# google-deepmind/bsuite

Measured on AMD Instinct MI355X. Metric: env-steps/sec, higher is better.
Workload: dtype int32; 1 GPU; deep_sea/10 deep_sea {'size': 30, 'mapping_seed': 42} random actions, dense TimeStep; mode=e, lanes_per_gpu=1048576, global_lanes=1048576, episode_phases=staggered

## Files before the change

bsuite_amd/_native.py:

```python
import ctypes
import os

import torch

_HERE = os.path.dirname(os.path.abspath(__file__))
SO_PATH = os.path.join(_HERE, '_lib', 'libbsuite_amd.so')

FIRST, MID, LAST = 0, 1, 2
BSX_EINVAL, BSX_ENULL, BSX_EALIGN, BSX_ERANGE, BSX_EMODE, BSX_ENOMEM = -1, -2, -3, -4, -5, -6
WRAP_NONE, WRAP_SCALE, WRAP_NOISE, WRAP_SCALE_NOISE, WRAP_NOISE_SCALE = 0, 1, 2, 3, 4
COUNTER_SHARDS, COUNTER_STRIDE = 256, 16
DEEP_SEA_MAX_SIZE = 64
BANDIT_MAX_ACTIONS = 32
FUSED_CATCH_MAX_CELLS = 128


class NativeLibraryError(RuntimeError):
  pass


def _load():
  override = os.environ.get('BSX_NATIVE_LIB')
  if override:
    try:
# ... 171 lines not shown


class ImageCfg(ctypes.Structure):
  _fields_ = [('mode', ctypes.c_int32), ('in_rows', ctypes.c_int32), ('in_cols', ctypes.c_int32),
              ('out_rows', ctypes.c_int32), ('out_cols', ctypes.c_int32), ('tail', ctypes.c_int32),
              ('radius_y', ctypes.c_int32), ('radius_x', ctypes.c_int32),
              ('gauss_y', ctypes.c_double * (IMAGE_MAX_RADIUS + 1)),
              ('gauss_x', ctypes.c_double * (IMAGE_MAX_RADIUS + 1))]


lib = _load()

_P = ctypes.c_void_p
_SIGS = {
    'bsx_abi_version': ([], ctypes.c_int),
    'bsx_observation_dtypes': ([ctypes.c_int32], ctypes.c_int),
    'bsx_observation_index_width': ([ctypes.c_int32], ctypes.c_int),
    'bsx_row_scratch_bytes': ([ctypes.c_int32, ctypes.c_int32, ctypes.c_int64], ctypes.c_int64),
    'bsx_bsuite_info': ([ctypes.c_int32, ctypes.c_int32, ctypes.c_int64, _P, _P, ctypes.c_int32, ctypes.c_int32, _P, _P],
                        ctypes.c_int),
    'bsx_lane_reset_mark': ([ctypes.c_int32, ctypes.c_int32, ctypes.c_int64, _P, _P, _P, ctypes.c_int32, _P], ctypes.c_int),
    'bsx_strerror': ([ctypes.c_int], ctypes.c_char_p),
    'bsx_calib_fill': ([_P, ctypes.c_int64, ctypes.c_int32, _P], ctypes.c_int),
    'bsx_calib_copy': ([_P, _P, ctypes.c_int64, ctypes.c_int32, _P], ctypes.c_int),
    'bsx_counter_add': ([_P, ctypes.c_uint64, _P], ctypes.c_int),
    'bsx_lambda_returns': ([ctypes.POINTER(Returns), _P], ctypes.c_int),
    'bsx_image_observation': ([ctypes.POINTER(ImageCfg), ctypes.c_int64, _P, _P, _P], ctypes.c_int),
    'bsx_image_observation_typed': ([ctypes.POINTER(ImageCfg), ctypes.c_int64, _P, ctypes.c_int32, _P, ctypes.c_int32,
                                     _P], ctypes.c_int),
    'bsx_stream_dump': ([ctypes.c_uint64, ctypes.c_uint64, ctypes.c_int64, ctypes.c_uint64,
                         ctypes.c_int32, ctypes.c_int32, _P, _P, _P], ctypes.c_int),
    'bsx_deep_sea_step': ([ctypes.POINTER(DeepSeaCfg), ctypes.POINTER(Call), _P, _P, TimeStepPtrs, _P],
                          ctypes.c_int),
    'bsx_catch_step': ([ctypes.POINTER(CatchCfg), ctypes.POINTER(Call), _P, _P, TimeStepPtrs, _P],
                       ctypes.c_int),
    'bsx_deep_sea_policy_rollout': ([ctypes.POINTER(DeepSeaCfg), ctypes.POINTER(Call), ctypes.POINTER(Policy), _P,
                                     TimeStepPtrs, _P], ctypes.c_int),
    'bsx_catch_policy_rollout': ([ctypes.POINTER(CatchCfg), ctypes.POINTER(Call), ctypes.POINTER(Policy), _P,
                                  TimeStepPtrs, _P], ctypes.c_int),
    'bsx_deep_sea_policy_evaluate': ([ctypes.POINTER(DeepSeaCfg), ctypes.POINTER(Call), ctypes.POINTER(Policy), _P,
                                      PolicyEvalPtrs, _P], ctypes.c_int),
    'bsx_catch_policy_evaluate': ([ctypes.POINTER(CatchCfg), ctypes.POINTER(Call), ctypes.POINTER(Policy), _P,
                                   PolicyEvalPtrs, _P], ctypes.c_int),
    'bsx_deep_sea_policy_sample': ([ctypes.POINTER(DeepSeaCfg), ctypes.POINTER(Call), ctypes.POINTER(PolicyLogits), _P,
                                    TimeStepPtrs, _P], ctypes.c_int),
    'bsx_catch_policy_sample': ([ctypes.POINTER(CatchCfg), ctypes.POINTER(Call), ctypes.POINTER(PolicyLogits), _P,
                                 TimeStepPtrs, _P], ctypes.c_int),
    'bsx_deep_sea_policy_sample_evaluate': ([ctypes.POINTER(DeepSeaCfg), ctypes.POINTER(Call), ctypes.POINTER(PolicyLogits), _P,
                                             PolicyEvalPtrs, _P], ctypes.c_int),
    'bsx_catch_policy_sample_evaluate': ([ctypes.POINTER(CatchCfg), ctypes.POINTER(Call), ctypes.POINTER(PolicyLogits), _P,
                                          PolicyEvalPtrs, _P], ctypes.c_int),
    'bsx_deep_sea_embedding_rollout': ([ctypes.POINTER(DeepSeaCfg), ctypes.POINTER(Call), ctypes.POINTER(PolicyEmbedding), _P,
                                        TimeStepPtrs, _P], ctypes.c_int),
    'bsx_catch_embedding_rollout': ([ctypes.POINTER(CatchCfg), ctypes.POINTER(Call), ctypes.POINTER(PolicyEmbedding), _P,
                                     TimeStepPtrs, _P], ctypes.c_int),
    'bsx_deep_sea_embedding_evaluate': ([ctypes.POINTER(DeepSeaCfg), ctypes.POINTER(Call), ctypes.POINTER(PolicyEmbedding), _P,
                                         PolicyEvalPtrs, _P], ctypes.c_int),
    'bsx_catch_embedding_evaluate': ([ctypes.POINTER(CatchCfg), ctypes.POINTER(Call), ctypes.POINTER(PolicyEmbedding), _P,
                                      PolicyEvalPtrs, _P], ctypes.c_int),
    'bsx_deep_sea_embedding_sample': ([ctypes.POINTER(DeepSeaCfg), ctypes.POINTER(Call), ctypes.POINTER(PolicyEmbeddingSample), _P,
                                       TimeStepPtrs, _P], ctypes.c_int),
    'bsx_catch_embedding_sample': ([ctypes.POINTER(CatchCfg), ctypes.POINTER(Call), ctypes.POINTER(PolicyEmbeddingSample), _P,
                                    TimeStepPtrs, _P], ctypes.c_int),
    'bsx_deep_sea_embedding_sample_evaluate': ([ctypes.POINTER(DeepSeaCfg), ctypes.POINTER(Call), ctypes.POINTER(PolicyEmbeddingSample),
                                                _P, PolicyEvalPtrs, _P], ctypes.c_int),
    'bsx_catch_embedding_sample_evaluate': ([ctypes.POINTER(CatchCfg), ctypes.POINTER(Call), ctypes.POINTER(PolicyEmbeddingSample), _P,
# ... 81 lines not shown
```

bsuite_amd/csrc/deep_sea.hip:

```cpp
#include "bsx_embed_device.h"
#include "bsx_pair_host.h"
#include "bsx_tab_eval.h"
#include "bsx_tab_sample_device.h"
#include "deep_sea_fam.h"
#include "pair_mixed.h"

template <int K>
__global__ void __launch_bounds__(BSX_BLOCK) deep_sea_step1_kernel(const deep_sea_fam::args a, const uint32_t cells,
                                                                   const uint32_t cells_magic, const bsx_div64 dv) {
  __shared__ deep_sea_fam::shared s_map[BSX_BLOCK / BSX_WAVE];
  const int wl = (int)(threadIdx.x & 63u);
  deep_sea_fam::shared& map = s_map[threadIdx.x >> 6];
  const int64_t n_lanes = a.ctl.n_lanes;
  const uint64_t step = bsx_step_of(a.ctl);
  const int32_t tag_new = (int32_t)(((uint32_t)(step + 1) & 1u) << DS_TAG_SHIFT);
  const bool forced = a.ctl.force_reset != 0;
  const deep_sea_hot fn{a.size};
  const uint64_t total = (uint64_t)n_lanes * cells;
  const uint64_t F0 = (uint64_t)blockIdx.x * (uint64_t)(K * 4 * BSX_BLOCK);
  const uint64_t lane_b = __umul64hi(F0, dv.m) >> dv.s;
  const uint32_t r_b = (uint32_t)(F0 - lane_b * cells);
  bsx_f4* __restrict__ o4 = reinterpret_cast<bsx_f4*>(a.out.observation + F0);
  const int32_t* __restrict__ st_b = a.state + lane_b;
  const int32_t* __restrict__ act_b = a.action + (forced ? 0 : lane_b);

  uint32_t dl[K];
  int r0[K];
  bool live[K];
#pragma unroll
  for (int u = 0; u < K; ++u) {
    const uint32_t c = (threadIdx.x >> 6) * (K * 64) + u * 64 + (threadIdx.x & 63);
    const uint32_t f = r_b + (c << 2);
    dl[u] = __umulhi(f, cells_magic);
    r0[u] = (int)(f - dl[u] * cells);
    live[u] = F0 + ((uint64_t)c << 2) + 3 < total;
  }
  const uint32_t dA = dl[0];
  uint32_t dB = dA;
  bool wrA = false, wrB = false;
#pragma unroll
  for (int u = 0; u < K; ++u) {
    if (live[u]) dB = dl[u];
  }
// ... 27 lines not shown
    return nst;
  };
  int tA = -1, tB = -1;
  int32_t nA = 0, nB = 0;
  if (any) {
    nA = resolve(dA, wA, aA, wrA, tA);
    nB = dB != dA ? resolve(dB, wB, aB, wrB, tB) : nA;
  }
  int hA, hB, unused;
  fn(nA, hA, unused);
  fn(nB, hB, unused);
#pragma unroll
  for (int u = 0; u < K; ++u) {
    if (!live[u]) continue;
    int hot = dl[u] == dA ? hA : hB;
    const int p0 = hot < 0 ? -1 : hot - r0[u];
    bsx_f4 v;
    v.x = p0 == 0 ? 1.0f : 0.0f;
    v.y = p0 == 1 ? 1.0f : 0.0f;
    v.z = p0 == 2 ? 1.0f : 0.0f;
    v.w = p0 == 3 ? 1.0f : 0.0f;
    o4[(threadIdx.x >> 6) * (K * 64) + u * 64 + (threadIdx.x & 63)] = v;
  }
  const unsigned int n_last = (unsigned int)__popcll(__ballot(tA == BSX_LAST)) + (unsigned int)__popcll(__ballot(tB == BSX_LAST));
  const unsigned int n_first = (unsigned int)__popcll(__ballot(tA == BSX_FIRST)) + (unsigned int)__popcll(__ballot(tB == BSX_FIRST));
  if (a.ctl.counters != nullptr && wl == 0 && (n_last | n_first) != 0u) {
    unsigned long long* shard = (unsigned long long*)a.ctl.counters +
                                (size_t)((blockIdx.x * (BSX_BLOCK / BSX_WAVE) + (threadIdx.x >> 6)) & (BSX_COUNTER_SHARDS - 1)) * BSX_COUNTER_STRIDE;
    if (n_last) atomicAdd(&shard[0], (unsigned long long)n_last);
    if (n_first) atomicAdd(&shard[1], (unsigned long long)n_first);
  }
}

static int deep_sea_check_cfg(const bsx_deep_sea_t* cfg) {
  return (cfg->size < 1 || cfg->size > BSX_DEEP_SEA_MAX_SIZE) ? BSX_ERANGE : 0;
}

static void deep_sea_fill(const bsx_deep_sea_t* cfg, const bsx_call_t* call, const int32_t* action, int32_t* state,
                          bsx_timestep_t out, double* info, deep_sea_fam::args* a) {
  a->ctl = bsx_make_ctl(call);
  a->action = action; a->state = state; a->out = out; a->info = info;
  a->move_cost = cfg->move_cost; a->inv_size = cfg->inv_size;
  a->size = cfg->size; a->deterministic = cfg->deterministic;
  for (int w = 0; w < DS_MAP_WORDS; ++w) a->mapping_bits[w] = cfg->mapping_bits[w];
}

static int deep_sea_make(const bsx_deep_sea_t* cfg, const bsx_call_t* call, const int32_t* action,
                         int32_t* state, bsx_timestep_t out, double* info, deep_sea_fam::args* a) {
  if (cfg == nullptr) return BSX_ENULL;
  int rc = bsx_check_call(call, action, out, true, true);
  if (rc != 0) return rc;
  if ((rc = deep_sea_check_cfg(cfg)) != 0) return rc;
  if (call->stream.mt_state != nullptr && !cfg->deterministic && call->stream.mt_gauss == nullptr)
    return BSX_ENULL;
  if (call->n_lanes > 0 && (state == nullptr || info == nullptr)) return BSX_ENULL;
  deep_sea_fill(cfg, call, action, state, out, info, a);
  return 0;
}

extern "C" int bsx_deep_sea_step(const bsx_deep_sea_t* cfg, const bsx_call_t* call,
                                 const int32_t* action, int32_t* state, bsx_timestep_t out,
                                 double* info) {
  deep_sea_fam::args a;
  int rc = deep_sea_make(cfg, call, action, state, out, info, &a);
  if (rc != 0) return rc;
  if (call->n_lanes == 0) return 0;
  const uint32_t cells = (uint32_t)(cfg->size * cfg->size);
  static const int step1_env = bsx_env_int("BSX_DEEP_SEA_STEP1", 1);
  if (step1_env != 0 && (int64_t)call->n_lanes * cells * 4 <= ((int64_t)1 << 30) && (call->flags & BSX_CALL_STATE_TAGGED) && call->n_steps <= 1 && call->action_ring <= 1 && cfg->deterministic && bsx_ctl_lean(a.ctl) &&
      call->obs_paint == nullptr && bsx_call_obs(call) == 0 && !bsx_call_index(call) && (cells & 3u) == 0 && cells >= 3u * 256u) {
    constexpr int K = 4;
    const uint64_t total = (uint64_t)call->n_lanes * cells;
    const uint64_t blocks = (total + (uint64_t)K * 4 * BSX_BLOCK - 1) / ((uint64_t)K * 4 * BSX_BLOCK);
    if (blocks > 0x7FFFFFFFull) return BSX_EINVAL;
    deep_sea_step1_kernel<K><<<dim3((unsigned)blocks), dim3(BSX_BLOCK), 0, (hipStream_t)call->hip_stream>>>(
        a, cells, bsx_div_magic(cells), bsx_make_div64(cells));
    return bsx_launch_status();
  }
  return bsx_pair_call<deep_sea_fam, deep_sea_hot, 4>(a, call, action, state, out, cells, deep_sea_hot{cfg->size});
}

extern "C" int bsx_deep_sea_policy_rollout(const bsx_deep_sea_t* cfg, const bsx_call_t* call, const bsx_policy_t* policy,
                                           int32_t* state, bsx_timestep_t out, double* info) {
  if (cfg == nullptr || call == nullptr || policy == nullptr) return BSX_ENULL;
  int rc = deep_sea_check_cfg(cfg);
  if (rc == 0) rc = bsx_check_policy_call(call, policy, bsx_policy_states_deep_sea(cfg->size), state, out, info);
  if (rc != 0 || call->n_lanes == 0) return rc;
  deep_sea_fam::args a;
  rc = deep_sea_make(cfg, call, policy->actions_out, state, out, info, &a);
  if (rc != 0) return rc;
  a.action = nullptr;
  return bsx_policy_rollout_call<deep_sea_fam, deep_sea_hot>(a, call, policy, 2u, out, deep_sea_hot{cfg->size});
}

extern "C" int bsx_deep_sea_policy_evaluate(const bsx_deep_sea_t* cfg, const bsx_call_t* call, const bsx_policy_t* policy,
                                             int32_t* state, bsx_policy_eval_t out, double* info) {
  if (cfg == nullptr || call == nullptr || policy == nullptr) return BSX_ENULL;
  int rc = deep_sea_check_cfg(cfg);
  if (rc == 0) rc = bsx_check_policy_eval_call(call, policy, bsx_policy_states_deep_sea(cfg->size), state, out, info);
  if (rc != 0 || call->n_lanes == 0) return rc;
  bsx_tab_eval_args e;
  deep_sea_fill(cfg, call, nullptr, state, bsx_timestep_t{}, info, &e.fam.deep_sea);
  return bsx_tab_eval_call(e, BSX_FAM_DEEP_SEA, call, policy, 2u, out);
}

extern "C" int bsx_deep_sea_policy_sample(const bsx_deep_sea_t* cfg, const bsx_call_t* call, const bsx_policy_logits_t* policy,
                                          int32_t* state, bsx_timestep_t out, double* info) {
  if (cfg == nullptr || call == nullptr || policy == nullptr) return BSX_ENULL;
  int rc = deep_sea_check_cfg(cfg);
  if (rc == 0) rc = bsx_check_tab_softmax_call(call, policy, bsx_policy_states_deep_sea(cfg->size), 2, state, out, info);
  if (rc != 0 || call->n_lanes == 0) return rc;
  bsx_tab_softmax_args s;
// ... 96 lines not shown
```

bsuite_amd/environments/base.py:

```python
import collections
import contextlib
import ctypes
import math
import secrets
from typing import Any, Dict, Optional

import numpy as np
import torch

from bsuite_amd import _native
from bsuite_amd import dm_env_compat as dm_env
from bsuite_amd.dm_env_compat import specs

_MASK63 = (1 << 63) - 1


_current_raw_stream = getattr(torch._C, '_cuda_getCurrentRawStream', None)
if _current_raw_stream is None:
  def _current_raw_stream(index):
    return torch.cuda.current_stream(index).cuda_stream
_current_device = getattr(torch._C, '_cuda_getDevice', None) or torch.cuda.current_device


_OBS_CODES = {torch.float32: 0, torch.uint8: 1, torch.float16: 2, torch.bfloat16: 3}
# ... 7 lines not shown

_MT_COLUMNS = ('state', 'pos', 'gauss', 'has_gauss')


PolicyEvaluation = collections.namedtuple('PolicyEvaluation', ['episodes', 'return_sum', 'episode_return_sum'])
LinearEvaluation = collections.namedtuple('LinearEvaluation', ['episodes', 'return_sum', 'episode_return_sum', 'observation'])


def raw(env):
  return env.raw_env if hasattr(env, 'raw_env') else env


def _timestep_ptrs(o) -> '_native.TimeStepPtrs':
  return _native.TimeStepPtrs(o['reward'].data_ptr(), o['discount'].data_ptr(), o['step_type'].data_ptr(),
                              o['observation'].data_ptr())


def _resolve_seed(seed: Optional[int]) -> int:
  if seed is None:
    return secrets.randbits(63)
  return int(seed) & _MASK63


class Environment(dm_env.EnvironmentBase):

  bsuite_num_episodes: int

  _supports_delta = False
  _supports_narrow_obs = False
  _index_width = 0
  _pipelined_rollout = False
  scalar_host_buffers = True
  row_path_min_bytes = None
  _state_tag_bit = None
  _state_lib_bits = 0
  _tag_calls = False
  _info_keys = ()
  _info_int_keys = ()
  _abi_name = None
  _cfg = None

  def __init__(self, obs_shape, num_actions, *, seed=None, batch=None, device=None,
               lane_offset=0, num_buffers=2, device_step_counter=False, shared_step_counter=None,
               rng='philox', observation_mode='dense', obs_allocator=None, observation_dtype=torch.float32):
    self._scalar = batch is None
    self._scalar_last_type = None
    self._batch = 1 if batch is None else int(batch)
    if self._batch < 1:
      raise ValueError('batch must be >= 1')
    self._device = torch.device('cuda:0' if device is None else device)
    if self._device.type == 'cuda' and self._device.index is None:
      self._device = torch.device('cuda', torch.cuda.current_device() if torch.cuda.is_available() else 0)
    self._lane_offset = int(lane_offset)
    self._seed = _resolve_seed(seed if seed is None or isinstance(seed, (int, np.integer)) else 0)
    self._obs_shape = tuple(int(d) for d in obs_shape)
    self._num_actions = int(num_actions)
    self._num_buffers = max(1, int(num_buffers))
    self._device_step_counter = bool(device_step_counter) or shared_step_counter is not None
    self._shared_step_counter = shared_step_counter
    self._obs_allocator = obs_allocator
    self._resolve_observations(observation_mode, observation_dtype)
    if rng not in ('philox', 'mt19937'):
      raise ValueError("rng must be 'philox' or 'mt19937'")
    self._rng_mode = rng
    self._mt_seeds = None
    if rng == 'mt19937':
      if seed is None or isinstance(seed, (int, np.integer)):
        self._mt_seeds = [(self._seed + i) & 0xFFFFFFFF for i in range(self._batch)]
      else:
        self._mt_seeds = [int(x) for x in seed]
        if len(self._mt_seeds) != self._batch:
          raise ValueError('need one seed per lane')
    self._wrap = (_native.WRAP_NONE, 0.0, 0, 0.0)
    self._wrap_mt_seeds = None
    self._wrap_mt = None
    self._logging = None
    self._deferred_steps = None
    self._grouped_by = None
    self._rollout_out = {}
    self._policy_rollout_out = {}
    self._policy_eval_out = None
    self._linear_eval_out = None
    self._state_alt = None
    self._row_buf = None
    self._dev_index = self._device.index
    self._step_index = 0
    self._buf = 0
    self._allocated = False
    self._reset_next_step = True

  def _resolve_observations(self, observation_mode, observation_dtype):
    if observation_mode not in ('dense', 'delta', 'index'):
      raise ValueError("observation_mode must be 'dense', 'delta' or 'index'")
    if observation_mode == 'delta' and not self._supports_delta:
      raise ValueError(f'{type(self).__name__} has no delta observation mode (its observations are small and dense)')
    self._delta = observation_mode == 'delta'
    self._index = observation_mode == 'index'
    self._board_shape = self._obs_shape
    if self._index:
      if not self._index_width:
        raise ValueError(f'{type(self).__name__} has no index observation mode (its observations are not one-hot boards)')
      if self._scalar:
        raise ValueError("observation_mode='index' needs the batched view (batch=B)")
      if self._obs_allocator is not None:
        raise ValueError("observation_mode='index' is not available in SweepBatch (float32 arenas)")
    dt = _OBS_NAMES.get(observation_dtype, observation_dtype) if isinstance(observation_dtype, str) else observation_dtype
    if dt not in _OBS_CODES:
      raise ValueError(f'observation_dtype must be one of {sorted(_OBS_NAMES)} (or the torch dtypes), got {observation_dtype!r}')
    if dt != torch.float32:
      if not self._supports_narrow_obs:
        raise ValueError(f'{type(self).__name__} writes float32 observations only (observation_dtype={observation_dtype!r})')
      if self._scalar:
        raise ValueError('observation_dtype other than float32 needs the batched view (batch=B)')
      if self._delta:
        raise ValueError("observation_dtype other than float32 needs observation_mode='dense'")
      if self._obs_allocator is not None:
        raise ValueError('observation_dtype other than float32 is not available in SweepBatch (float32 arenas)')
# ... 59 lines not shown

  def _state_tensors(self) -> Dict[str, torch.Tensor]:
    raise NotImplementedError

  def _native_args(self, call, action_ptr, out):
    state = tuple(t.data_ptr() for t in self._state.values())
    info = (self._info.data_ptr(),) if self._info_keys else ()
    return (ctypes.byref(self._cfg), ctypes.byref(call), action_ptr) + state + (out,) + info

  def _launch(self, call, action_ptr, out) -> int:
    return getattr(_native.lib, f'bsx_{self._abi_name}_step')(*self._native_args(call, action_ptr, out))

  def _group_set(self, group, index: int, action: torch.Tensor, *, out=None, state_alt=None,
                 swap_state: bool = False, row_scratch=None) -> int:
    if self._index:
      raise ValueError("grouped launches write dense observations; use observation_mode='dense'")
    self._ensure_allocated()
    ring = int(action.shape[0]) if (torch.is_tensor(action) and action.dim() == 2) else 0
    if (not torch.is_tensor(action) or action.dtype != torch.int32 or action.device != self._device
        or tuple(action.shape) not in ((self._batch,), (ring, self._batch)) or not action.is_contiguous()
        or (action.dim() == 2 and (ring < 1 or ring & (ring - 1)))):
      raise ValueError(f'grouped launches read the action tensor in place every step: need a contiguous int32 '
                       f'tensor of shape ({self._batch},) — or an action ring (R, {self._batch}) with R a power '
                       f'of two — on {self._device}')
    if not self._device_step_counter:
      raise ValueError('grouped launches need device_step_counter / shared_step_counter')
    if self._delta:
      raise ValueError("grouped launches write dense observations; use observation_mode='dense'")
    if self._obs_flags:
      raise ValueError('grouped launches write float32 observations; use observation_dtype=torch.float32')
    call = self._call_desc
    call.force_reset, call.n_steps = 0, 0
    self._sync_wrap()
    call.stream.step_index = 0
    call.action_ring = ring
    self._buf = 1 % self._num_buffers
    ptrs = self._out_ptrs[0] if out is None else _timestep_ptrs(out)
    own = self._state.get('state')
    own_rows = call.row_scratch
    if row_scratch is not None:
      call.row_scratch = row_scratch.data_ptr() if row_scratch is not False else None
    try:
      if state_alt is not None:
        if swap_state:
          self._state['state'], call.state_alt = state_alt, own.data_ptr()
        else:
          call.state_alt = state_alt.data_ptr()
      return getattr(_native.lib, f'bsx_group_set_{self._abi_name}')(
          group, index, *self._native_args(call, action.data_ptr(), ptrs))
    finally:
      call.state_alt = None
      call.action_ring = 0
      call.row_scratch = own_rows
      if state_alt is not None:
        self._state['state'] = own

  def _row_scratch_words(self) -> int:
    fam = _native.FAMILY_IDS.get(self._abi_name, -1)
    return int(_native.lib.bsx_row_scratch_bytes(fam, int(np.prod(self._obs_shape)), self._batch)) // 4 if fam >= 0 else 0

  def _row_scratch(self, fresh: bool = False) -> Optional[torch.Tensor]:
    words = self._row_scratch_words()
    if not words:
      return None
    if fresh or self._row_buf is None:
      with torch.cuda.device(self._device):
# ... 67 lines not shown
      self._scalar_action = torch.zeros(1, dtype=torch.int32, **place)
      self._reward_f64 = torch.zeros(1, dtype=torch.float64, **place) if self._scalar else None
      self._out_np = [{k: v.numpy() for k, v in o.items()} for o in self._out] if self._host_out else None
    self._mt = None
    if self._rng_mode == 'mt19937':
      with torch.cuda.device(dev):
        self._mt = self._mt_columns(self._mt_seeds, dev, prepare=self._mt_constructor_draws)
    mt_ptrs = [self._mt[k].data_ptr() if self._mt else None for k in _MT_COLUMNS]
    self._call_desc = _native.Call(
        n_lanes=B, force_reset=0,
        stream=_native.Stream(self._seed, self._lane_offset, 0,
                              self._step_base.data_ptr() if self._device_step_counter else None,
                              *mt_ptrs),
        wrap=_native.RewardWrap(_native.WRAP_NONE, 0, 0.0, 0, None, None, None, None, 0.0),
        counters=self._counters.data_ptr(), hip_stream=None)
    if self._reward_f64 is not None:
      self._call_desc.reward_f64 = self._reward_f64.data_ptr()
    if (not self._scalar and self.row_path_min_bytes is not None and self._row_scratch_words()
        and B * int(np.prod(self._obs_shape)) * 4 >= self.row_path_min_bytes):
      self._call_desc.row_scratch = self._row_scratch().data_ptr()
    if self._wrap_mt_seeds is not None:
      self._upload_wrap_mt()
    self._fn = getattr(_native.lib, f'bsx_{self._abi_name}_step')
    self._family_id = _native.FAMILY_IDS[self._abi_name]
    self._reset_column = 'steps' if 'steps' in self._state else 'state'
    self._argv = [list(self._native_args(self._call_desc, 0, p)) for p in self._out_ptrs]
    self._call_stream, self._call_wrap = self._call_desc.stream, self._call_desc.wrap
    self._wrap_applied = None
    if self._state_tag_bit is not None:
      self._tag_calls = self._shared_step_counter is None
      self._call_desc.flags = _native.CALL_STATE_TAGGED if self._tag_calls else 0
    self._call_desc.flags |= self._obs_flags
    self._tag_host_count = self._tag_calls and not self._device_step_counter
    self._allocated = True

  def _new_outputs(self, lead, place, observation=None):
    o = dict(reward=torch.empty(lead, dtype=torch.float32, **place),
             discount=torch.empty(lead, dtype=torch.float32, **place),
             step_type=torch.empty(lead, dtype=torch.int8, **place),
             observation=(observation if observation is not None else
                          torch.empty(tuple(lead) + self._obs_shape, dtype=self._obs_dtype, **place)))
    return o, _timestep_ptrs(o), dm_env.TimeStep(step_type=o['step_type'], reward=o['reward'], discount=o['discount'],
                                                 observation=o['observation'])

  def _sync_wrap(self):
    w = self._call_desc.wrap
    w.kind, w.param, w.seed, w.param2 = self._wrap
    self._wrap_applied = self._wrap

  def _redirected(self, method, *args):
    with torch.cuda.device(self._device):
      return method(*args)

  def _call(self, action_ptr: int, force_reset: bool) -> int:
    if _current_device() != self._dev_index:
      return self._redirected(self._call, action_ptr, force_reset)
    b = self._buf
    self._buf = b + 1 if b + 1 < self._num_buffers else 0
    call = self._call_desc
    if self._delta:
      call.obs_paint = self._paint[b].data_ptr()
    call.force_reset = 1 if force_reset else 0
    if self._tag_host_count:
      call.flags = (0 if torch.cuda.is_current_stream_capturing() else _native.CALL_STATE_TAGGED) | self._obs_flags
    if self._wrap is not self._wrap_applied:
      w = self._call_wrap
      w.kind, w.param, w.seed, w.param2 = self._wrap
      self._wrap_applied = self._wrap
    hip_stream = _current_raw_stream(self._dev_index)
    call.hip_stream = hip_stream
    argv = self._argv[b]
    argv[2] = action_ptr
    if self._device_step_counter:
      if self._deferred_steps is not None:
        self._call_stream.step_index = self._deferred_steps
        rc = self._fn(*argv)
        self._call_stream.step_index = 0
        self._deferred_steps += 1
      else:
        rc = self._fn(*argv)
        if rc == 0 and self._shared_step_counter is None:
          rc = _native.lib.bsx_counter_add(self._step_base.data_ptr(), 1, hip_stream)
    else:
      self._call_stream.step_index = self._step_index
      rc = self._fn(*argv)
    if rc != 0:
      _native.check(rc, f'{type(self).__name__} step')
    self._step_index += 1
    return b

  def _launch_steps(self, fn, args, T: int, what: str):
    if _current_device() != self._dev_index:
      return self._redirected(self._launch_steps, fn, args, T, what)
    call = self._call_desc
    call.force_reset, call.n_steps = 0, T
    self._sync_wrap()
    hip_stream = _current_raw_stream(self._dev_index)
    call.hip_stream = hip_stream
    call.stream.step_index = 0 if self._device_step_counter else self._step_index
    try:
      rc = fn(*args)
      if rc == 0 and self._device_step_counter and self._shared_step_counter is None:
        rc = _native.lib.bsx_counter_add(self._step_base.data_ptr(), T, hip_stream)
    finally:
      call.n_steps = 0
      call.state_alt = None
    if rc != 0:
      _native.check(rc, f'{type(self).__name__} {what}')
    self._step_index += T
    return None

  def enable_logging(self, log_by_step: bool = False, log_every: bool = False,
                     max_rows: Optional[int] = None, max_count: Optional[int] = None):
    from bsuite_amd.utils import wrappers as _w
    if self._grouped_by is not None:
      raise RuntimeError('enable_logging() on a segment of prepared sweep groups: SweepBatch.release_groups() first')
    self._ensure_allocated()
    if self._logging is None:
      for j, pending in self._pending_info().items():
        self._info[j] += pending
      self._clear_pending_info()
    explicit_count = max_count is not None
    if max_count is None:
      max_count = 10 ** 18
    points = _w.logarithmic_logging_points(max_count)
    if max_rows is None:
      if self._scalar:
        max_rows = 8
      elif log_every:
        max_rows = 4096
      else:
        horizon = max_count if explicit_count else (
            max(10 ** 4, 100 * int(getattr(self, 'bsuite_num_episodes', 0) or 0)) * (1000 if log_by_step else 1))
        max_rows = (2 if log_by_step else 1) * sum(1 for p_ in points if p_ <= horizon) + 2
    B, dev = self._batch, self._device
    n_info = len(self._info_keys)
    place = dict(pin_memory=True) if self._host_out else dict(device=dev)
    lg = {k: torch.zeros(B, dtype=torch.float64 if k.endswith('_return') else torch.int64, **place)
          for k in LOGGING_COLUMNS}
    lg.update(rows=torch.zeros((B, max_rows, len(LOGGING_COLUMNS) + n_info), dtype=torch.float64, **place),
              n_rows=torch.zeros(B, dtype=torch.int32, **place),
              log_points=torch.tensor(points, dtype=torch.int64, device=dev))
    self._logging = lg
    self._logging_desc = _native.Logging(
        info=self._info.data_ptr() if n_info else None, **{k: v.data_ptr() for k, v in lg.items()},
        n_log_points=len(points), max_rows=max_rows,
        n_info=n_info, log_by_step=int(bool(log_by_step)), log_every=int(bool(log_every)))
    self._call_desc.logging = ctypes.pointer(self._logging_desc)
    return lg

# ... 51 lines not shown

  def step(self, action, reset_mask=None) -> dm_env.TimeStep:
    if not self._allocated:
      if reset_mask is not None:
        self._check_reset_mask(reset_mask)
      self._ensure_allocated()
    if reset_mask is None and (
        type(action) is torch.Tensor and action.dtype is torch.int32 and action.is_cuda and action.dim() == 1
        and action.size(0) == self._batch and action.is_contiguous() and action.get_device() == self._dev_index
        and not self._scalar):
      ptr = action.data_ptr()
    else:
      if reset_mask is not None:
        self._check_reset_mask(reset_mask)
      ptr = self._coerce_actions(action).data_ptr()
      if reset_mask is not None:
        self._mark_reset(reset_mask)
    return self._wrap_output(self._call(ptr, force_reset=False))

  def _check_reset_mask(self, mask):
    if self._scalar:
      raise ValueError('reset_mask / mark_reset() need the batched view (batch=B); reset() is the one lane of the '
                       'scalar view')
    if self._grouped_by is not None:
      raise RuntimeError('mark_reset() on a segment of prepared sweep groups: SweepBatch.release_groups() first')
    if (not torch.is_tensor(mask) or mask.dtype not in (torch.bool, torch.uint8) or mask.device != self._device
        or tuple(mask.shape) != (self._batch,) or not mask.is_contiguous()):
      raise ValueError(f'reset_mask must be a contiguous bool or uint8 tensor of shape ({self._batch},) on '
                       f'{self._device}')

  def _mark_reset(self, mask):
    if _current_device() != self._dev_index:
      return self._redirected(self._mark_reset, mask)
    col = self._info_pending_column
    folded = 1 if (self._logging is None and col is not None) else 0
    rc = _native.lib.bsx_lane_reset_mark(
        self._family_id, self._info_variant, self._batch, mask.data_ptr(),
        self._state[self._reset_column].data_ptr(), self._info.data_ptr(), folded, _current_raw_stream(self._dev_index))
    if rc != 0:
      _native.check(rc, f'{type(self).__name__} mark_reset')
    return None

  def mark_reset(self, mask):
    self._check_reset_mask(mask)
    self._ensure_allocated()
    self._mark_reset(mask)

  def rollout(self, actions) -> dm_env.TimeStep:
    if self._scalar:
      raise TypeError('rollout() needs the batched view (batch=B)')
    if self._delta:
      raise ValueError("rollout() writes T separate observation arrays; use observation_mode='dense'")
    self._ensure_allocated()
    if not torch.is_tensor(actions) or actions.dim() != 2 or actions.shape[1] != self._batch:
      raise ValueError(f'expected actions of shape (T, {self._batch})')
    if actions.device != self._device or actions.dtype != torch.int32:
      actions = actions.to(device=self._device, dtype=torch.int32)
    actions = actions.contiguous()
    T = int(actions.shape[0])
    if T < 1:
      raise ValueError('rollout needs at least one step')
    if T not in self._rollout_out:
      self._rollout_out[T] = self._new_outputs((T, self._batch), dict(device=self._device))
    _, ptrs, timestep = self._rollout_out[T]
    call = self._call_desc
    if self._pipelined_rollout and T > 1 and not self._index:
# ... 554 lines not shown

  def episode_counters(self) -> torch.Tensor:
    self._ensure_allocated()
    return self._counters[:, :2].sum(dim=0)

  def invalid_action_count(self) -> torch.Tensor:
    self._ensure_allocated()
    return self._counters[:, 2].sum()

  def state_dict(self) -> Dict[str, Any]:
    self._ensure_allocated()
    d = {k: v.clone() for k, v in self._state.items()}
    if self._state_lib_bits:
      d['state'] &= ~self._state_lib_bits
    d['__info'] = self._info.clone()
    d['__counters'] = self._counters.clone()
    d['__step_index'] = self.device_step_index()
    d['__seed'] = self._seed
    if self._rng_mode == 'mt19937':
      for k, v in self._mt.items():
        d['__mt_' + k] = v.clone()
      if self._wrap_mt is not None:
        for k, v in self._wrap_mt.items():
          d['__wrap_mt_' + k] = v.clone()
    d['__wrap'] = tuple(self._wrap)
    if self._logging is not None:
      for k in LOGGING_COLUMNS + ('rows', 'n_rows'):
        d['__logging_' + k] = self._logging[k].clone()
    return d

  def load_state_dict(self, d: Dict[str, Any]):
    self._ensure_allocated()
    self._scalar_last_type = None
    for k, v in self._state.items():
      v.copy_(d[k])
    self._info.copy_(d['__info'])
    self._counters.copy_(d['__counters'])
    self._step_index = int(d['__step_index'])
    if self._state_tag_bit is not None:
      st = self._state['state']
      st &= ~self._state_lib_bits
      if self._step_index & 1:
        st |= self._state_tag_bit
    if self._device_step_counter:
      self._step_base.fill_(self._step_index)
    self._seed = int(d['__seed'])
    self._call_desc.stream.seed = self._seed
    if self._rng_mode == 'mt19937':
      for k, v in self._mt.items():
        v.copy_(d['__mt_' + k])
      if self._wrap_mt is not None:
        for k, v in self._wrap_mt.items():
          v.copy_(d['__wrap_mt_' + k])
    if '__wrap' in d:
      self._wrap = (tuple(d['__wrap']) + (0.0,))[:4]
    has_log = '__logging_steps' in d
    if has_log != (self._logging is not None):
      raise ValueError('state_dict was taken %s the Logging wrapper but this environment runs %s it: '
                       'wrap (or unwrap) the environment before load_state_dict'
                       % (('with', 'without') if has_log else ('without', 'with')))
    if has_log:
      if d['__logging_rows'].shape != self._logging['rows'].shape:
        raise ValueError('Logging row buffers differ in shape (max_rows): construct Logging with the same max_rows')
      for k in LOGGING_COLUMNS + ('rows', 'n_rows'):
        self._logging[k].copy_(d['__logging_' + k])
```

bsuite_amd/environments/deep_sea.py:

```python
import warnings
from typing import Optional

import numpy as np
import torch

from bsuite_amd import _native
from bsuite_amd.environments import base

NUM_EPISODES = 10000


class DeepSea(base.Environment):

  _info_keys = ('total_bad_episodes', 'denoised_return')
  _info_int_keys = ('total_bad_episodes',)

  def __init__(self,
               size: int,
               deterministic: bool = True,
               unscaled_move_cost: float = 0.01,
               randomize_actions: bool = True,
               seed: Optional[int] = None,
               mapping_seed: Optional[int] = None,
               **engine_kwargs):
# ... 11 lines not shown
      warnings.warn('Environment is in debug mode (randomize_actions=False).'
                    'Only randomized_actions=True is the DeepSea environment.')
      self._action_mapping = np.ones([size, size])

    if not self._deterministic:
      optimal_no_cost = (1 - 1 / self._size) ** (self._size - 1)
    else:
      optimal_no_cost = 1.
    self._optimal_return = optimal_no_cost - self._unscaled_move_cost

    cfg = _native.DeepSeaCfg()
    cfg.size = size
    cfg.deterministic = int(bool(deterministic))
    cfg.move_cost = float(unscaled_move_cost) / size
    cfg.inv_size = 1 / size
    flat = np.asarray(self._action_mapping).reshape(-1) == 1
    for idx in np.nonzero(flat)[0]:
      cfg.mapping_bits[int(idx) >> 5] |= (1 << (int(idx) & 31))
    self._cfg = cfg
    self.bsuite_num_episodes = NUM_EPISODES

  def _state_tensors(self):
    return dict(state=torch.full((self._batch,), 1 << 17, dtype=torch.int32, device=self._device))

  _abi_name = 'deep_sea'
  _supports_delta = True
  _supports_narrow_obs = True
  _index_width = 1
  _pipelined_rollout = True

  _state_tag_bit = 1 << 18
  _state_lib_bits = 1 << 18

  _policy_abi = 'bsx_deep_sea_policy_rollout'
  _policy_eval_abi = 'bsx_deep_sea_policy_evaluate'
  _policy_sample_abi = 'bsx_deep_sea_policy_sample'
  _policy_sample_eval_abi = 'bsx_deep_sea_policy_sample_evaluate'
  _embedding_rollout_abi = 'bsx_deep_sea_embedding_rollout'
  _embedding_eval_abi = 'bsx_deep_sea_embedding_evaluate'
  _embedding_sample_abi = 'bsx_deep_sea_embedding_sample'
  _embedding_sample_eval_abi = 'bsx_deep_sea_embedding_sample_evaluate'

  @property
  def policy_num_states(self) -> int:
    return self._size * self._size

  @property
  def optimal_return(self):
    return self._optimal_return
```

include/bsuite_amd.h:

```cpp
#ifndef BSUITE_AMD_H_
#define BSUITE_AMD_H_

#include <stdint.h>

#ifdef __cplusplus
extern "C" {
#endif

#define BSX_ABI_VERSION 12

#define BSX_FIRST 0
#define BSX_MID 1
#define BSX_LAST 2

#define BSX_EINVAL (-1)
#define BSX_ENULL (-2)
#define BSX_EALIGN (-3)
#define BSX_ERANGE (-4)
#define BSX_EMODE (-5)
#define BSX_ENOMEM (-6)

typedef struct {
  uint64_t seed;
  uint64_t lane_offset;
// ... 63 lines not shown
  double* reward_f64;
  int32_t* state_alt;
  int32_t action_ring;
  int32_t flags;
  void* row_scratch;
} bsx_call_t;

#define BSX_CALL_STATE_TAGGED 1
#define BSX_CALL_OBS_SHIFT 1
#define BSX_CALL_OBS_MASK (3 << BSX_CALL_OBS_SHIFT)
#define BSX_CALL_OBS_F32 (0 << BSX_CALL_OBS_SHIFT)
#define BSX_CALL_OBS_U8 (1 << BSX_CALL_OBS_SHIFT)
#define BSX_CALL_OBS_F16 (2 << BSX_CALL_OBS_SHIFT)
#define BSX_CALL_OBS_BF16 (3 << BSX_CALL_OBS_SHIFT)

#define BSX_CALL_OBS_INDEX (1 << 3)

int bsx_observation_index_width(int32_t family);

int bsx_observation_dtypes(int32_t family);

#define BSX_FUSED_CATCH_MAX_CELLS 128

#define BSX_DEEP_SEA_MAX_SIZE 64
typedef struct {
  int32_t size;
  int32_t deterministic;
  double move_cost;
  double inv_size;
  uint32_t mapping_bits[BSX_DEEP_SEA_MAX_SIZE * BSX_DEEP_SEA_MAX_SIZE / 32];
} bsx_deep_sea_t;
int bsx_deep_sea_step(const bsx_deep_sea_t* cfg , const bsx_call_t* call ,
                      const int32_t* action, int32_t* state, bsx_timestep_t out, double* info);

typedef struct {
  int32_t rows;
  int32_t columns;
} bsx_catch_t;
int bsx_catch_step(const bsx_catch_t* cfg, const bsx_call_t* call, const int32_t* action,
                   int32_t* state, bsx_timestep_t out, double* info);

typedef struct {
  const uint8_t* table;
  int32_t n_states, n_policies;
  const int32_t* policy_index;
  double epsilon;
  uint64_t explore_seed;
  int32_t* actions_out;
} bsx_policy_t;
int bsx_deep_sea_policy_rollout(const bsx_deep_sea_t* cfg, const bsx_call_t* call, const bsx_policy_t* policy,
                                int32_t* state, bsx_timestep_t out, double* info);
int bsx_catch_policy_rollout(const bsx_catch_t* cfg, const bsx_call_t* call, const bsx_policy_t* policy,
                             int32_t* state, bsx_timestep_t out, double* info);

typedef struct { int32_t* episodes; double* return_sum; double* episode_return_sum; } bsx_policy_eval_t;
int bsx_deep_sea_policy_evaluate(const bsx_deep_sea_t* cfg, const bsx_call_t* call, const bsx_policy_t* policy,
                                 int32_t* state, bsx_policy_eval_t out, double* info);
int bsx_catch_policy_evaluate(const bsx_catch_t* cfg, const bsx_call_t* call, const bsx_policy_t* policy,
                              int32_t* state, bsx_policy_eval_t out, double* info);

typedef struct {
  const float*   logits;
  int32_t        n_states, n_actions, n_policies;
  const int32_t* policy_index;
  double         inv_temperature;
  uint64_t       sample_seed;
// ... 296 lines not shown
```

Measured before the change: 1.768 billion env-steps/s.

## Split deep_sea step into state-advance and hint-driven observation streaming roles

Adds a hinted deep_sea step. One set of blocks advances lane state and writes a packed per-lane hint: the two candidate next hot cells plus the mapping bit. Within the same launch, the remaining blocks paint the one-hot observation from the previous step's hint and the current action, so they never decode state. This separates the small state update from the large observation write and lets both run concurrently in one grid. The cost is an extra hint buffer, a fallback launch on the first call, and host-side bookkeeping that invalidates the hint on resets, wrappers, logging and state loads.

After: 1.816 billion env-steps/s (median of 6 runs). +2.8%, better.

```diff
diff --git a/bsuite_amd/_native.py b/bsuite_amd/_native.py
--- a/bsuite_amd/_native.py
+++ b/bsuite_amd/_native.py
@@ -227,6 +227,8 @@
                          ctypes.c_int32, ctypes.c_int32, _P, _P, _P], ctypes.c_int),
     'bsx_deep_sea_step': ([ctypes.POINTER(DeepSeaCfg), ctypes.POINTER(Call), _P, _P, TimeStepPtrs, _P],
                           ctypes.c_int),
+    'bsx_deep_sea_step_hinted': ([ctypes.POINTER(DeepSeaCfg), ctypes.POINTER(Call), _P, _P, TimeStepPtrs, _P, _P, _P],
+                                 ctypes.c_int),
     'bsx_catch_step': ([ctypes.POINTER(CatchCfg), ctypes.POINTER(Call), _P, _P, TimeStepPtrs, _P],
                        ctypes.c_int),
     'bsx_deep_sea_policy_rollout': ([ctypes.POINTER(DeepSeaCfg), ctypes.POINTER(Call), ctypes.POINTER(Policy), _P,
diff --git a/bsuite_amd/csrc/deep_sea.hip b/bsuite_amd/csrc/deep_sea.hip
--- a/bsuite_amd/csrc/deep_sea.hip
+++ b/bsuite_amd/csrc/deep_sea.hip
@@ -3,12 +3,29 @@
 #include "bsx_tab_eval.h"
 #include "bsx_tab_sample_device.h"
 #include "deep_sea_fam.h"
+#include "deep_sea_hint.h"
 #include "pair_mixed.h"
+
+__device__ __forceinline__ void deep_sea_hint_advance(const deep_sea_fam::args& a, uint32_t block_id, uint32_t* __restrict__ hint_out,
+                                                      deep_sea_fam::shared& s_fam, unsigned int* s_cnt);
+template <int K>
+__device__ __forceinline__ void deep_sea_hint_stream(float* __restrict__ obs, const uint32_t* __restrict__ hint_in,
+                                                     const int32_t* __restrict__ action, int64_t n_lanes, uint32_t cells,
+                                                     uint32_t cells_magic, bsx_div64 dv, uint32_t block_id);
 
 template <int K>
 __global__ void __launch_bounds__(BSX_BLOCK) deep_sea_step1_kernel(const deep_sea_fam::args a, const uint32_t cells,
-                                                                   const uint32_t cells_magic, const bsx_div64 dv) {
+                                                                   const uint32_t cells_magic, const bsx_div64 dv,
+                                                                   const uint32_t adv_blocks, const uint32_t* __restrict__ hint_in,
+                                                                   uint32_t* __restrict__ hint_out) {
   __shared__ deep_sea_fam::shared s_map[BSX_BLOCK / BSX_WAVE];
+  if (hint_out != nullptr) {
+    __shared__ unsigned int s_cnt[2];
+    const bsx_pipe_role r = bsx_pipe_role_of(blockIdx.x, gridDim.x, adv_blocks, 0u);
+    if (r.adv) deep_sea_hint_advance(a, r.index, hint_out, s_map[0], s_cnt);
+    else deep_sea_hint_stream<K>(a.out.observation, hint_in, a.action, a.ctl.n_lanes, cells, cells_magic, dv, r.index);
+    return;
+  }
   const int wl = (int)(threadIdx.x & 63u);
   deep_sea_fam::shared& map = s_map[threadIdx.x >> 6];
   const int64_t n_lanes = a.ctl.n_lanes;
@@ -102,6 +119,82 @@
   }
 }
 
+__device__ __forceinline__ void deep_sea_hint_advance(const deep_sea_fam::args& a, uint32_t block_id, uint32_t* __restrict__ hint_out,
+                                                      deep_sea_fam::shared& s_fam, unsigned int* s_cnt) {
+  if (threadIdx.x < 2) s_cnt[threadIdx.x] = 0;
+  deep_sea_fam::stage(a, s_fam);
+  __syncthreads();
+  const uint64_t step = bsx_step_of(a.ctl);
+  int64_t i[2];
+  bool mine[2];
+  int act[2], type[2] = {-1, -1};
+  int32_t st[2];
+#pragma unroll
+  for (int h = 0; h < 2; ++h) {
+    i[h] = (int64_t)block_id * (2 * BSX_BLOCK) + h * BSX_BLOCK + threadIdx.x;
+    mine[h] = i[h] < a.ctl.n_lanes;
+    act[h] = 0; st[h] = 0;
+    if (mine[h]) {
+      act[h] = a.action[i[h]];
+      st[h] = a.state[i[h]];
+    }
+  }
+#pragma unroll
+  for (int h = 0; h < 2; ++h) {
+    if (mine[h]) {
+      const uint64_t lane = a.ctl.lane_offset + (uint64_t)i[h];
+      int32_t nst; double reward;
+      type[h] = deep_sea_fam::advance<true, 1>(a, s_fam, i[h], lane, step, st[h], act[h], nst, reward);
+      a.state[i[h]] = nst;
+      hint_out[i[h]] = ds_hint_pack(nst & 0xFF, (nst >> 8) & 0xFF, nst & DS_RESET_BIT, a.size, s_fam.map);
+      bsx_emit_at<0, 0, false>(a.ctl, a.out, i[h], i[h], lane, step, type[h], reward);
+    }
+    bsx_count_types(a.ctl, type[h], s_cnt);
+  }
+  bsx_final_barrier();
+  bsx_flush_counts(a.ctl, s_cnt, block_id);
+}
+
+template <int K>
+__device__ __forceinline__ void deep_sea_hint_stream(float* __restrict__ obs, const uint32_t* __restrict__ hint_in,
+                                                     const int32_t* __restrict__ action, int64_t n_lanes, uint32_t cells,
+                                                     uint32_t cells_magic, bsx_div64 dv, uint32_t block_id) {
+  const uint64_t total = (uint64_t)n_lanes * cells;
+  const uint64_t F0 = (uint64_t)block_id * (uint64_t)(K * 4 * BSX_BLOCK);
+  const uint64_t lane_b = __umul64hi(F0, dv.m) >> dv.s;
+  const uint32_t r_b = (uint32_t)(F0 - lane_b * cells);
+  bsx_f4* __restrict__ o4 = reinterpret_cast<bsx_f4*>(obs + F0);
+  const uint32_t* __restrict__ hi = hint_in + lane_b;
+  const int32_t* __restrict__ ac = action + lane_b;
+
+  int r0[K];
+  uint32_t h0[K];
+  int32_t a0[K];
+  bool live[K];
+#pragma unroll
+  for (int u = 0; u < K; ++u) {
+    const uint32_t c = (threadIdx.x >> 6) * (K * 64) + u * 64 + (threadIdx.x & 63);
+    const uint32_t f = r_b + (c << 2);
+    const uint32_t dl = __umulhi(f, cells_magic);
+    r0[u] = (int)(f - dl * cells);
+    live[u] = F0 + ((uint64_t)c << 2) + 3 < total;
+    h0[u] = live[u] ? hi[dl] : 0u;
+    a0[u] = live[u] ? ac[dl] : 0;
+  }
+#pragma unroll
+  for (int u = 0; u < K; ++u) {
+    if (!live[u]) continue;
+    const int hot = ds_hint_hot(h0[u], a0[u]);
+    const int p0 = hot < 0 ? -1 : hot - r0[u];
+    bsx_f4 v;
+    v.x = p0 == 0 ? 1.0f : 0.0f;
+    v.y = p0 == 1 ? 1.0f : 0.0f;
+    v.z = p0 == 2 ? 1.0f : 0.0f;
+    v.w = p0 == 3 ? 1.0f : 0.0f;
+    o4[(threadIdx.x >> 6) * (K * 64) + u * 64 + (threadIdx.x & 63)] = v;
+  }
+}
+
 static int deep_sea_check_cfg(const bsx_deep_sea_t* cfg) {
   return (cfg->size < 1 || cfg->size > BSX_DEEP_SEA_MAX_SIZE) ? BSX_ERANGE : 0;
 }
@@ -144,10 +237,37 @@
     const uint64_t blocks = (total + (uint64_t)K * 4 * BSX_BLOCK - 1) / ((uint64_t)K * 4 * BSX_BLOCK);
     if (blocks > 0x7FFFFFFFull) return BSX_EINVAL;
     deep_sea_step1_kernel<K><<<dim3((unsigned)blocks), dim3(BSX_BLOCK), 0, (hipStream_t)call->hip_stream>>>(
-        a, cells, bsx_div_magic(cells), bsx_make_div64(cells));
+        a, cells, bsx_div_magic(cells), bsx_make_div64(cells), 0u, nullptr, nullptr);
     return bsx_launch_status();
   }
   return bsx_pair_call<deep_sea_fam, deep_sea_hot, 4>(a, call, action, state, out, cells, deep_sea_hot{cfg->size});
+}
+
+extern "C" int bsx_deep_sea_step_hinted(const bsx_deep_sea_t* cfg, const bsx_call_t* call, const int32_t* action, int32_t* state,
+                                        bsx_timestep_t out, double* info, const uint32_t* const hint_in, uint32_t* const hint_out) {
+  if (cfg == nullptr || call == nullptr) return BSX_ENULL;
+  if ((reinterpret_cast<uintptr_t>(out.observation) & 15u) != 0) return BSX_EMODE;
+  deep_sea_fam::args a;
+  int rc = deep_sea_make(cfg, call, action, state, out, info, &a);
+  if (rc != 0) return rc;
+  const uint32_t cells = (uint32_t)(cfg->size * cfg->size);
+  if (!cfg->deterministic || !bsx_ctl_lean(a.ctl) || bsx_call_obs(call) != 0 || bsx_call_index(call) || call->obs_paint != nullptr ||
+      call->n_steps > 1 || call->action_ring > 1 || call->force_reset != 0 || !(call->flags & BSX_CALL_STATE_TAGGED) || (cells & 3u) != 0)
+    return BSX_EMODE;
+  if (call->n_lanes == 0) return 0;
+  if (hint_out == nullptr || hint_out == hint_in) return BSX_ENULL;
+  hipStream_t st = (hipStream_t)call->hip_stream;
+  const uint64_t adv_blocks = (uint64_t)((bsx_blocks_of(call->n_lanes) + 1) / 2);
+  const uint64_t str_blocks = hint_in == nullptr ? 0 : bsx_flat_blocks((uint64_t)call->n_lanes * cells, PAIR_DEEP_SEA_K);
+  if (adv_blocks + str_blocks > 0x7FFFFFFFull) return BSX_EINVAL;
+  const uint32_t magic = bsx_div_magic(cells);
+  deep_sea_step1_kernel<PAIR_DEEP_SEA_K><<<dim3((unsigned)(adv_blocks + str_blocks)), dim3(BSX_BLOCK), 0, st>>>(
+      a, cells, magic, bsx_make_div64(cells), (uint32_t)adv_blocks, hint_in, hint_out);
+  if (hint_in == nullptr) {
+    rc = bsx_launch_hot_stream<deep_sea_hot, PAIR_DEEP_SEA_K>(out.observation, state, call->n_lanes, cells, magic, deep_sea_hot{cfg->size}, st);
+    if (rc != 0) return rc;
+  }
+  return bsx_launch_status();
 }
 
 extern "C" int bsx_deep_sea_policy_rollout(const bsx_deep_sea_t* cfg, const bsx_call_t* call, const bsx_policy_t* policy,
diff --git a/bsuite_amd/csrc/deep_sea_hint.h b/bsuite_amd/csrc/deep_sea_hint.h
--- /dev/null
+++ b/bsuite_amd/csrc/deep_sea_hint.h
@@ -0,0 +1,38 @@
+#ifndef BSX_DEEP_SEA_HINT_H_
+#define BSX_DEEP_SEA_HINT_H_
+
+#include <stdint.h>
+
+#include "../../include/bsuite_amd.h"
+#include "../../include/bsx_stream.h"
+
+#define DS_HINT_FIELD_BITS 13
+#define DS_HINT_FIELD_MASK ((1u << DS_HINT_FIELD_BITS) - 1u)
+#define DS_HINT_L_SHIFT DS_HINT_FIELD_BITS
+#define DS_HINT_M_SHIFT (2 * DS_HINT_FIELD_BITS)
+
+#if BSX_DEEP_SEA_MAX_SIZE * BSX_DEEP_SEA_MAX_SIZE + 1 > (1 << DS_HINT_FIELD_BITS)
+#error "a hint field must hold every hot cell + 1"
+#endif
+
+BSX_HD uint32_t ds_hint_pack(int row, int col, int reset_pending, int N, const uint32_t* mapping_bits) {
+  if (reset_pending) return 1u | (1u << DS_HINT_L_SHIFT);
+  if ((unsigned)row >= (unsigned)N || (unsigned)col >= (unsigned)N) return 0u;
+  const int cell = row * N + col;
+  const uint32_t m = (mapping_bits[cell >> 5] >> (cell & 31)) & 1u;
+  uint32_t r = 0u, l = 0u;
+  if (row + 1 < N) {
+    const int base = (row + 1) * N + 1;
+    r = (uint32_t)(base + (col + 1 > N - 1 ? N - 1 : col + 1));
+    l = (uint32_t)(base + (col - 1 < 0 ? 0 : col - 1));
+  }
+  return r | (l << DS_HINT_L_SHIFT) | (m << DS_HINT_M_SHIFT);
+}
+
+BSX_HD int ds_hint_hot(uint32_t hint, int32_t action) {
+  const int32_t m = (int32_t)((hint >> DS_HINT_M_SHIFT) & 1u);
+  const uint32_t f = action == m ? hint : hint >> DS_HINT_L_SHIFT;
+  return (int)(f & DS_HINT_FIELD_MASK) - 1;
+}
+
+#endif
diff --git a/bsuite_amd/environments/base.py b/bsuite_amd/environments/base.py
--- a/bsuite_amd/environments/base.py
+++ b/bsuite_amd/environments/base.py
@@ -63,6 +63,7 @@
   _pipelined_rollout = False
   scalar_host_buffers = True
   row_path_min_bytes = None
+  hint_min_bytes = None
   _state_tag_bit = None
   _state_lib_bits = 0
   _tag_calls = False
@@ -114,6 +115,12 @@
     self._linear_eval_out = None
     self._state_alt = None
     self._row_buf = None
+    self._hint_ok = False
+    self._hint_valid = False
+    self._hint = None
+    self._hint_cur = 0
+    self._hint_argv = None
+    self.hint_launches = [0, 0, 0]
     self._dev_index = self._device.index
     self._step_index = 0
     self._buf = 0
@@ -239,6 +246,7 @@
     call = self._call_desc
     call.force_reset, call.n_steps = 0, 0
     self._sync_wrap()
+    self._hint_ok = False
     call.stream.step_index = 0
     call.action_ring = ring
     self._buf = 1 % self._num_buffers
@@ -372,7 +380,28 @@
       self._call_desc.flags = _native.CALL_STATE_TAGGED if self._tag_calls else 0
     self._call_desc.flags |= self._obs_flags
     self._tag_host_count = self._tag_calls and not self._device_step_counter
+    self._hint_ok = (self.hint_min_bytes is not None and self._tag_calls and self._hint_static_ok()
+                     and B * int(np.prod(self._obs_shape)) * 4 > self.hint_min_bytes)
     self._allocated = True
+
+  def _hint_static_ok(self) -> bool:
+    return False
+
+  def _hinted_call(self, b: int, action_ptr: int):
+    if self._hint is None:
+      self._hint = torch.empty((2, self._batch), dtype=torch.int32, device=self._device)
+      self._hint_fn = getattr(_native.lib, f'bsx_{self._abi_name}_step_hinted')
+      self._hint_ptrs = (self._hint[0].data_ptr(), self._hint[1].data_ptr())
+      self._hint_argv = [a + [None, None] for a in self._argv]
+    argv = self._hint_argv[b]
+    argv[2] = action_ptr
+    cur = self._hint_cur
+    argv[-2] = self._hint_ptrs[cur] if self._hint_valid else None
+    argv[-1] = self._hint_ptrs[1 - cur]
+    self.hint_launches[0 if self._hint_valid else 1] += 1
+    self._hint_cur = 1 - cur
+    self._hint_valid = False
+    return self._hint_fn, argv
 
   def _new_outputs(self, lead, place, observation=None):
     o = dict(reward=torch.empty(lead, dtype=torch.float32, **place),
@@ -387,6 +416,7 @@
     w = self._call_desc.wrap
     w.kind, w.param, w.seed, w.param2 = self._wrap
     self._wrap_applied = self._wrap
+    self._hint_valid = False
 
   def _redirected(self, method, *args):
     with torch.cuda.device(self._device):
@@ -407,25 +437,36 @@
       w = self._call_wrap
       w.kind, w.param, w.seed, w.param2 = self._wrap
       self._wrap_applied = self._wrap
+      self._hint_valid = False
     hip_stream = _current_raw_stream(self._dev_index)
     call.hip_stream = hip_stream
-    argv = self._argv[b]
+    fn, argv = self._fn, self._argv[b]
     argv[2] = action_ptr
+    hinted = False
+    if self._hint_ok:
+      if (force_reset or self._logging is not None or self._wrap[0] >= _native.WRAP_NOISE or self._grouped_by is not None
+          or call.action_ring > 1 or torch.cuda.is_current_stream_capturing()):
+        self._hint_valid = False
+        self.hint_launches[2] += 1
+      else:
+        fn, argv = self._hinted_call(b, action_ptr)
+        hinted = True
     if self._device_step_counter:
       if self._deferred_steps is not None:
         self._call_stream.step_index = self._deferred_steps
-        rc = self._fn(*argv)
+        rc = fn(*argv)
         self._call_stream.step_index = 0
         self._deferred_steps += 1
       else:
-        rc = self._fn(*argv)
+        rc = fn(*argv)
         if rc == 0 and self._shared_step_counter is None:
           rc = _native.lib.bsx_counter_add(self._step_base.data_ptr(), 1, hip_stream)
     else:
       self._call_stream.step_index = self._step_index
-      rc = self._fn(*argv)
+      rc = fn(*argv)
     if rc != 0:
       _native.check(rc, f'{type(self).__name__} step')
+    self._hint_valid = hinted
     self._step_index += 1
     return b
 
@@ -456,6 +497,7 @@
     if self._grouped_by is not None:
       raise RuntimeError('enable_logging() on a segment of prepared sweep groups: SweepBatch.release_groups() first')
     self._ensure_allocated()
+    self._hint_valid = False
     if self._logging is None:
       for j, pending in self._pending_info().items():
         self._info[j] += pending
@@ -573,6 +615,7 @@
   def _mark_reset(self, mask):
     if _current_device() != self._dev_index:
       return self._redirected(self._mark_reset, mask)
+    self._hint_valid = False
     col = self._info_pending_column
     folded = 1 if (self._logging is None and col is not None) else 0
     rc = _native.lib.bsx_lane_reset_mark(
@@ -1193,6 +1236,7 @@
   def load_state_dict(self, d: Dict[str, Any]):
     self._ensure_allocated()
     self._scalar_last_type = None
+    self._hint_valid = False
     for k, v in self._state.items():
       v.copy_(d[k])
     self._info.copy_(d['__info'])
diff --git a/bsuite_amd/environments/deep_sea.py b/bsuite_amd/environments/deep_sea.py
--- a/bsuite_amd/environments/deep_sea.py
+++ b/bsuite_amd/environments/deep_sea.py
@@ -67,6 +67,12 @@
   _state_tag_bit = 1 << 18
   _state_lib_bits = 1 << 18
 
+  hint_min_bytes = 1 << 30
+
+  def _hint_static_ok(self) -> bool:
+    return (bool(self._deterministic) and (self._size * self._size) % 4 == 0 and not self._scalar and not self._delta
+            and not self._index and not self._obs_flags and self._rng_mode == 'philox')
+
   _policy_abi = 'bsx_deep_sea_policy_rollout'
   _policy_eval_abi = 'bsx_deep_sea_policy_evaluate'
   _policy_sample_abi = 'bsx_deep_sea_policy_sample'
diff --git a/include/bsuite_amd.h b/include/bsuite_amd.h
--- a/include/bsuite_amd.h
+++ b/include/bsuite_amd.h
@@ -119,6 +119,9 @@
 } bsx_deep_sea_t;
 int bsx_deep_sea_step(const bsx_deep_sea_t* cfg , const bsx_call_t* call ,
                       const int32_t* action, int32_t* state, bsx_timestep_t out, double* info);
+
+int bsx_deep_sea_step_hinted(const bsx_deep_sea_t* cfg, const bsx_call_t* call, const int32_t* action, int32_t* state,
+                             bsx_timestep_t out, double* info, const uint32_t* hint_in, uint32_t* hint_out);
 
 typedef struct {
   int32_t rows;
```
